# leggedrobotics/open3d_slam

Measured on AMD Instinct MI355X. Metric: icp_iterations_per_sec, higher is better.
Workload: dtype f32 points, f64 accumulate; 1 GPU; configs[1]: point-to-plane ICP, 65536-pt VLP-16 scan vs a 1,000,000-pt submap, max_corr 1.0 m, 10 fixed iterations/step (+1 evaluation pass), index prebuilt; n_src=65536, n_map_per_gpu=1000000, parallelism=1 GPU

## Files before the change

open3d_slam_amd/csrc/backend.hip:

```cpp
#include <hip/hip_runtime.h>
#include <sched.h>

#include <algorithm>
#include <atomic>
#include <chrono>
#include <cmath>
#include <cstdio>
#include <cstdlib>
#include <climits>
#include <cstring>
#include <initializer_list>
#include <map>

#include <rocprim/device/device_radix_sort.hpp>
#include <mutex>
#include <string>
#include <type_traits>
#include <unordered_map>
#include <vector>

#include "cloud_kernels.hpp"
#include "common.hpp"
#include "feature_kernels.hpp"
#include "icp_kernels.hpp"
// ... 10 lines not shown
#ifdef O3DS_AB_SWITCHES
inline const char* ab_getenv(const char* name) { return getenv(name); }
#else
inline const char* ab_getenv(const char*) { return nullptr; }
#endif

struct CloudRec {
  size_t n = 0;
  int precision = 0;
  void* pts = nullptr;
  void* nrm = nullptr;
  void* col = nullptr;
  size_t cap = 0;
  bool has_index = false;
  bool index_byproduct = false;
  GridDev grid{};
  int* cell_start = nullptr;
  void* spts = nullptr;
  void* snrm = nullptr;
  void* rpts = nullptr;
  int* rstart = nullptr;
  int* rpos = nullptr;
  int index_regs = 0;
  long long vox_first = -1;
  size_t vox_count = 0;
  struct PMapRec* pm = nullptr;
  size_t index_positions = 0;
  int lazy_slot = -1;
  int lazy_seq = 0;
  size_t n_lower = 0;
  hipEvent_t ingest_ev = nullptr;
  int ingest_buf = -1;
  int pre_slot = -1;
  int pre_seq = 0;
  CropDev pre_crop{};
  bool has_box = false;
  bool box_padded = false;
  double bmn[3] = {0, 0, 0}, bmx[3] = {0, 0, 0};
  double* fpfh = nullptr;
  bool has_fpfh = false;
  size_t fpfh_n = 0;
};

void box_inflate(CloudRec& c) {
  if (c.box_padded) return;
  c.box_padded = true;
// ... 31 lines not shown
  }
  for (int a = 0; a < 3; ++a)
    if (!std::isfinite(to.bmn[a]) || !std::isfinite(to.bmx[a])) to.has_box = false;
  if (to.has_box) box_inflate(to);
}

struct PMapRec {
  PmDev dev{};
  CropDev* d_hist = nullptr;
  int t = 0;
  size_t n_upper = 0;
  size_t live_lower = 0;
  double clamped = 0;
  double multi_total = 0;
  double pool_top = 0;
  int rec_slot = -1, rec_seq = 0;
  size_t rows = 0;
  std::vector<void*> blocks;
};

constexpr int kMaxPassBlocks = 4096;
constexpr size_t kMaxCells = (size_t)1 << 27;
constexpr size_t kReplicaMaxBytes = (size_t)256 << 20;
static_assert(kReplicaMaxBytes <= kScanMaxBytes, "scan_strided addresses a searched array by 32-bit byte offsets");

}

struct DenseRec {
  double voxel = 0.0;
  size_t cap = 0;
  o3ds::DenseDev dev{};
  bool has_normals = false;
  bool has_colors = false;
  size_t used_upper = 0;
};

struct o3ds_context {
  int device = 0;
  hipStream_t stream = nullptr;
  int precision = O3DS_PRECISION_F32;
  std::string err, deferred_err;
  std::unordered_map<uint64_t, CloudRec> clouds;
  std::unordered_map<uint64_t, DenseRec> dense_maps;
  uint64_t next_id = 1;
  double* d_partials = nullptr;
  IcpStateDev* d_state = nullptr;
// ... 355 lines not shown
}
CloudRec* find_cloud(o3ds_handle h, o3ds_cloud id) {
  auto it = h->clouds.find(id);
  if (it == h->clouds.end()) return nullptr;
  cloud_ready(h, it->second);
  if (resolve_count(h, it->second, true) != O3DS_OK || (it->second.pm && pm_exit(h, it->second) != O3DS_OK)) {
    h->deferred_err = h->err;
    return nullptr;
  }
  return &it->second;
}

void free_index(o3ds_handle h, CloudRec& c) {
  if (c.cell_start) dev_free(h, c.cell_start);
  if (c.spts) dev_free(h, c.spts);
  if (c.snrm) dev_free(h, c.snrm);
  if (c.rpts) dev_free(h, c.rpts);
  if (c.rstart) dev_free(h, c.rstart);
  if (c.rpos) dev_free(h, c.rpos);
  c.cell_start = nullptr;
  c.spts = c.snrm = c.rpts = nullptr;
  c.rstart = c.rpos = nullptr;
  c.index_regs = 0;
  c.has_index = false;
  c.index_byproduct = false;
}
constexpr int kPinRecs = 64;
inline int* cnt_word(o3ds_handle h, int slot) { return h->d_cnt + 16 * slot; }
int resolve_count(o3ds_handle h, CloudRec& c, bool block);

constexpr uint64_t kRecOwnerMap = ~0ull - 1;
int take_rec(o3ds_handle h) {
  for (int tries = 0; tries < kPinRecs; ++tries) {
    const int slot = h->rec_next;
    h->rec_next = (h->rec_next + 1) % kPinRecs;
    if (h->rec_owner[slot] == 0) {
      h->rec_owner[slot] = ~0ull;
      return slot;
    }
  }
  for (int tries = 0; tries < kPinRecs; ++tries) {
    const int slot = h->rec_next;
    h->rec_next = (h->rec_next + 1) % kPinRecs;
    auto it = h->clouds.find(h->rec_owner[slot]);
    if (it == h->clouds.end()) continue;
    if (it->second.lazy_slot == slot && resolve_count(h, it->second, true) != O3DS_OK) continue;
// ... 299 lines not shown
template <typename P4>
int bbox_of(o3ds_handle h, const P4* pts, size_t n, double mn[3], double mx[3], const CropDev* crop = nullptr) {
  const int g = grid_for(n, 1024);
  static_assert(1024 * 6 * sizeof(double) <= kPinBytes - 256, "bbox partials fit the pinned block");
  CropDev all{};
  bbox_kernel<P4><<<g, kBlock, 0, h->stream>>>(pts, n, crop ? *crop : all, (double*)h->h_pin_dev);
  HIP_TRY(hipGetLastError());
  HIP_TRY(hipStreamSynchronize(h->stream));
  const double* hb = (const double*)h->h_pin;
  for (int a = 0; a < 3; ++a) {
    mn[a] = 1e300;
    mx[a] = -1e300;
  }
  for (int b = 0; b < g; ++b)
    for (int a = 0; a < 3; ++a) {
      mn[a] = std::min(mn[a], hb[(size_t)b * 6 + a]);
      mx[a] = std::max(mx[a], hb[(size_t)b * 6 + 3 + a]);
    }
  return O3DS_OK;
}

template <typename P4>
int build_grid_t(o3ds_handle h, const P4* pts, const P4* nrm, size_t n, double cell, GridDev* out_grid, int** out_cell_start, void** out_spts,
                 void** out_snrm, CloudRec* box ,
                 const int* n_dev = nullptr ) {
  if (n == 0) return fail(h, O3DS_ERR_EMPTY, "build_index: empty cloud");
  if (n > kScanMaxBytes / sizeof(P4))
    return fail(h, O3DS_ERR_CAPACITY, "build_index: the cell-sorted points exceed 2^32 bytes (2^28 points in f32 storage, 2^27 in f64): the search addresses them by 32-bit byte offsets");
  double mn[3], mx[3];
  int rc = O3DS_OK;
  static const bool no_box_cache = ab_getenv("O3DS_NO_BOX_CACHE") != nullptr;
  if (box && box->has_box && !no_box_cache) {
    for (int a = 0; a < 3; ++a) mn[a] = box->bmn[a], mx[a] = box->bmx[a];
  } else {
    if (n_dev) return fail(h, O3DS_ERR_INVALID_ARG, "build_index: a cloud whose size is still in flight must bring its box");
    rc = bbox_of<P4>(h, pts, n, mn, mx);
    if (rc) return rc;
    if (box) {
      box->has_box = true;
      box->box_padded = false;
      for (int a = 0; a < 3; ++a) box->bmn[a] = mn[a], box->bmx[a] = mx[a];
    }
  }
  for (int a = 0; a < 3; ++a)
    if (!std::isfinite(mn[a]) || !std::isfinite(mx[a])) return fail(h, O3DS_ERR_INVALID_ARG, "build_index: non-finite coordinates");
  size_t nx, ny, nz;
  for (;;) {
    nx = (size_t)std::floor((mx[0] - mn[0]) / cell) + 1;
    ny = (size_t)std::floor((mx[1] - mn[1]) / cell) + 1;
    nz = (size_t)std::floor((mx[2] - mn[2]) / cell) + 1;
    if (nx * ny * nz <= kMaxCells) break;
    cell *= 1.26;
  }
  const size_t ncell = nx * ny * nz;
  GridDev g{};
  g.ox = mn[0];
  g.oy = mn[1];
  g.oz = mn[2];
  g.cell = cell;
  g.inv_cell = 1.0 / cell;
  g.nx = (int)nx;
  g.sx = (int)nx;
  g.ny = (int)ny;
  g.nz = (int)nz;
  int *counts = nullptr, *cell_id = nullptr, *cell_start = nullptr;
  void *spts = nullptr, *snrm = nullptr;
  rc = cell_counters(h, ncell);
  if (rc) return rc;
  if (!h->d_cells) return fail(h, O3DS_ERR_OOM, "build_index: cell counters allocation failed");
  counts = h->d_cells;
  TMP_ALLOC(cell_id, sizeof(int) * n);
  HIP_TRY(dev_alloc(h, (void**)&cell_start, sizeof(int) * (ncell + 1 + 4)));
  HIP_TRY(dev_alloc(h, (void**)&spts, sizeof(P4) * n));
  if (nrm) HIP_TRY(dev_alloc(h, (void**)&snrm, sizeof(P4) * n));
  span_mark(h, kSpanIndexBuild);
  cell_count_kernel<P4><<<grid_for(n), kBlock, 0, h->stream>>>(pts, n, g, counts, cell_id, n_dev);
  rc = exclusive_scan_int(h, counts, cell_start, ncell + 1);
  if (rc) return rc;
  scatter_kernel<P4><<<grid_for(n), kBlock, 0, h->stream>>>(pts, nrm, n, cell_id, cell_start, counts, (P4*)spts, (P4*)snrm, n_dev);
  span_mark(h, kSpanIndexBuild);
  HIP_TRY(hipGetLastError());
  h->cells_clean = true;
  dbg_sync(h, 2);
  g.cell_start = cell_start;
  *out_grid = g;
  *out_cell_start = cell_start;
  *out_spts = spts;
  if (out_snrm) *out_snrm = snrm;
  return O3DS_OK;
}

template <typename P4>
int build_index_t(o3ds_handle h, CloudRec& c, double cell) {
  free_index(h, c);
  if (c.lazy_slot >= 0 && !c.has_box) {
    const int rr = resolve_count(h, c, true);
    if (rr) return rr;
  }
  int rc = build_grid_t<P4>(h, (const P4*)c.pts, (const P4*)c.nrm, c.n, cell, &c.grid, &c.cell_start, &c.spts, &c.snrm, &c,
                            c.lazy_slot >= 0 ? cnt_word(h, c.lazy_slot) : nullptr);
  if (rc) return rc;
  c.has_index = true;
  return O3DS_OK;
}

double index_cell_div() {
  static const double d = ab_getenv("O3DS_INDEX_CELL_DIV") ? std::max(1.0, atof(ab_getenv("O3DS_INDEX_CELL_DIV"))) : 4.0;
  return d;
}

int build_index(o3ds_handle h, CloudRec& c, double cell) { return DISPATCH(c.precision, build_index_t, h, c, cell); }

template <typename P4>
int build_replica_t(o3ds_handle h, CloudRec& c) {
  GridDev g = c.grid;
  const size_t n = c.n, rcell = (size_t)g.nx * (size_t)(g.ny + 2) * (size_t)(g.nz + 2);
  if (rcell > kMaxCells || 9 * n > (size_t)INT_MAX || 9 * n * (sizeof(P4) + sizeof(int)) + sizeof(int) * (rcell + 1) > kReplicaMaxBytes) return O3DS_OK;
  void* rpts = nullptr;
  int *rstart = nullptr, *rpos = nullptr;
  if (dev_alloc(h, (void**)&rstart, sizeof(int) * (rcell + 1)) != hipSuccess || dev_alloc(h, &rpts, sizeof(P4) * 9 * n) != hipSuccess ||
      dev_alloc(h, (void**)&rpos, sizeof(int) * 9 * n) != hipSuccess) {
    (void)hipGetLastError();
    if (rstart) dev_free(h, rstart);
    if (rpts) dev_free(h, rpts);
    return O3DS_OK;
  }
  const int rs = cell_counters(h, rcell);
  if (rs || !h->d_cells) {
    (void)hipGetLastError();
    dev_free(h, rstart), dev_free(h, rpts), dev_free(h, rpos);
    return rs;
  }
  int* rcounts = h->d_cells;
  const int* n_dev = c.lazy_slot >= 0 ? cnt_word(h, c.lazy_slot) : nullptr;
  replica_count_kernel<P4><<<grid_for(n), kBlock, 0, h->stream>>>((const P4*)c.spts, n, g, rcounts, n_dev);
  const int rc = exclusive_scan_int(h, rcounts, rstart, rcell + 1);
  if (rc) {
    dev_free(h, rstart), dev_free(h, rpts), dev_free(h, rpos);
    return rc;
  }
  replica_scatter_kernel<P4><<<grid_for(n), kBlock, 0, h->stream>>>((const P4*)c.spts, n, g, rstart, rcounts, (P4*)rpts, rpos, n_dev);
  HIP_TRY(hipGetLastError());
  h->cells_clean = true;
  c.rpts = rpts;
  c.rstart = rstart;
  c.rpos = rpos;
  c.grid.rpts = rpts;
  c.grid.rstart = rstart;
  c.grid.rpos = rpos;
  return O3DS_OK;
}

constexpr int kReplicaAfterRegs = 4;
int maybe_build_replica(o3ds_handle h, CloudRec& c) {
  if (!c.has_index || c.rpts || c.pm || c.index_positions) return O3DS_OK;
  const char* e = ab_getenv("O3DS_NN_REPLICA_AFTER");
  const int after = e ? std::max(1, atoi(e)) : kReplicaAfterRegs;
  if (++c.index_regs < after) return O3DS_OK;
  return DISPATCH(c.precision, build_replica_t, h, c);
}

int h2d_copy_narrow(o3ds_handle h, float* d_dst, const double* h_src, size_t count) {
  int rc = stage_init(h);
  if (rc) return rc;
  const size_t per = kStageBytes / sizeof(float);
  int k = 0;
  for (size_t off = 0; off < count; off += per, k ^= 1) {
// ... 373 lines not shown
    int e = 0;
    (void)std::frexp(nn * bound[k], &e);
    q_hi[k] = no_split ? 0.0 : std::ldexp(1.0, e + 3 - 53);
  }
}

int begin_session(o3ds_handle h, o3ds_cloud source, o3ds_cloud target, const o3ds_crop* crop, const double init[16],
                  const o3ds_icp_params* params, bool upload_state = true) {
  CloudRec* src = find_cloud_lazy(h, source);
  CloudRec* tgt = find_cloud_lazy(h, target);
  if (src && src->pm) {
    const int re = pm_exit(h, *src);
    if (re) return re;
    tgt = find_cloud_lazy(h, target);
  }
  int rc = validate_icp(h, src, tgt, params);
  if (rc) return rc;
  const double r_hint = params->max_correspondence_distance;
  static const double reuse_max = ab_getenv("O3DS_INDEX_REUSE_MAX") ? atof(ab_getenv("O3DS_INDEX_REUSE_MAX")) : 0.75;
  if (!tgt->has_index || (tgt->nrm && !tgt->snrm) || (tgt->index_byproduct && (tgt->grid.cell < r_hint / 8.0 || tgt->grid.cell > r_hint * reuse_max))) {
    rc = build_index(h, *tgt, params->max_correspondence_distance / index_cell_div());
    if (rc) return rc;
  }
  const size_t cap = (std::max<size_t>(src->n + src->n / 4, 1 << 16) + 7) & ~(size_t)7;
  bool fresh_cache = false;
  rc = handle_scratch(h, &h->d_nn_cache, &h->nn_cache_cap, src->n, cap, cap * sizeof(int), &fresh_cache);
  if (rc) return rc;
  if (!h->d_nn_cache) return fail(h, O3DS_ERR_OOM, "icp: match cache allocation failed");
  if (fresh_cache) {
    if (h->d_set_pos) (void)hipFree(h->d_set_pos);
    h->d_set_pos = nullptr;
    h->d_set_ref = nullptr;
    if (hipMalloc((void**)&h->d_set_pos, cap * (kSetCap * sizeof(int) + 4 * sizeof(double))) != hipSuccess) {
      (void)hipFree(h->d_nn_cache);
      h->d_nn_cache = nullptr;
      h->nn_cache_cap = 0;
      return fail(h, O3DS_ERR_OOM, "icp: candidate-set allocation failed");
    }
    h->d_set_ref = (char*)h->d_set_pos + cap * kSetCap * sizeof(int);
  }
  IcpStateDev st{};
  memcpy(st.T, init, sizeof(double) * 16);
  *h->h_state = st;
  if (upload_state) HIP_TRY(hipMemcpyAsync(h->d_state, h->h_state, sizeof(IcpStateDev), hipMemcpyHostToDevice, h->stream));
  IcpPassArgs a{};
  a.src = src->pts;
  a.first = 0;
  a.count = src->n;
  a.tpts = tgt->spts;
  a.tnrm = tgt->snrm;
  rc = maybe_build_replica(h, *tgt);
  if (rc) return rc;
  a.grid = tgt->grid;
  {
    const char* e = ab_getenv("O3DS_NN_REPLICA");
    if (e && atoi(e) == 0) a.grid.rpts = nullptr, a.grid.rstart = a.grid.rpos = nullptr;
  }
  a.crop = to_dev(crop);
  const double r = params->max_correspondence_distance;
  a.r2max = r * r;
  a.method = params->method;
  record_quanta(tgt->grid, r, params->method, h->gicp_epsilon, src->n, a.q_hi);
  a.kmax = std::max(1, (int)std::ceil(r / tgt->grid.cell));
  a.nn_cache = h->d_nn_cache;
  a.set_pos = h->fused && h->sets ? h->d_set_pos : nullptr;
  a.set_ref = h->d_set_ref;
  a.set_gain = h->set_gain;
  a.set_min = h->set_min;
  a.set_cap = h->set_cap;
  a.n_tgt = (int)(tgt->index_positions ? tgt->index_positions : tgt->n);
  a.snrm = src->nrm;
  a.count_dev = src->lazy_slot >= 0 ? cnt_word(h, src->lazy_slot) : nullptr;
  a.gicp_k = 1.0 - h->gicp_epsilon;
  a.state = h->d_state;
  a.partials = h->d_partials;
// ... 1420 lines not shown
    std::vector<unsigned long long> ws((size_t)o3ds::kNrmStatWords * ((size_t)o3ds::kNrmWaves * gsz));
    HIP_TRY(hipMemcpy(ws.data(), d_ws, sizeof(unsigned long long) * ws.size(), hipMemcpyDeviceToHost));
    (void)hipFree(d_ws);
    if (FILE* f = fopen(sf, "wb")) {
      fwrite(ws.data(), sizeof(unsigned long long), ws.size(), f);
      fclose(f);
    }
  }
#endif
  if (nrm_debug) {
    fprintf(stderr, "[normals] kernel done: %s\n", hipGetErrorString(hipStreamSynchronize(h->stream)));
#ifdef O3DS_NRM_CHECK
    unsigned int dbg[8] = {0};
    (void)hipMemcpyFromSymbol(dbg, HIP_SYMBOL(o3ds::g_nrm_dbg), sizeof(dbg));
    fprintf(stderr, "[normals] violations: unsorted %u, bad p %u, bad oi %u\n", dbg[0], dbg[1], dbg[2]);
    const unsigned int zero[8] = {0};
    (void)hipMemcpyToSymbol(HIP_SYMBOL(o3ds::g_nrm_dbg), zero, sizeof(zero));
#endif
  }
  tmp.pts = nullptr;
  box_copy(c, tmp);
  free_index(h, c);
  c.grid = tmp.grid, c.cell_start = tmp.cell_start, c.spts = tmp.spts, c.snrm = tmp.snrm;
  c.has_index = true;
  c.index_byproduct = true;
  return O3DS_OK;
}

int gicp_knn_normals(o3ds_handle h, CloudRec& c) {
  return DISPATCH(c.precision, normals_t, h, c, 0.0, 20, true);
}

template <typename P4>
int transform_t(o3ds_handle h, const CloudRec& in, const double T[16], CloudRec& out) {
  out.precision = in.precision;
  out.n = in.n;
  box_transform(out, in, T);
  if (in.n == 0) return O3DS_OK;
  HIP_TRY(dev_alloc(h, (void**)&out.pts, sizeof(P4) * in.n));
  if (in.nrm) HIP_TRY(dev_alloc(h, (void**)&out.nrm, sizeof(P4) * in.n));
  transform_kernel<P4><<<grid_for(in.n), kBlock, 0, h->stream>>>((const P4*)in.pts, (const P4*)in.nrm, in.n, mat34(T), T[3], T[7], T[11], T[15],
                                                               (P4*)out.pts, (P4*)out.nrm, 0);
  if (in.col) {
    HIP_TRY(dev_alloc(h, (void**)&out.col, sizeof(P4) * in.n));
    HIP_TRY(hipMemcpyAsync(out.col, in.col, sizeof(P4) * in.n, hipMemcpyDeviceToDevice, h->stream));
  }
// ... 666 lines not shown
    if ((double)gn[0] * (double)gn[1] * (double)gn[2] <= (double)kMaxCells / 2 && gn[0] < 5000) break;
    d.kc *= 2;
    cell = d.kc * voxel;
  }
  for (int a = 0; a < 3; ++a)
    if (std::llabs(g0[a]) + gn[a] * d.kc >= (1ll << 20)) return fail(h, O3DS_ERR_INVALID_ARG, "persistent map: voxel coordinates beyond 2^20");
  d.gx0 = g0[0], d.gy0 = g0[1], d.gz0 = g0[2];
  GridDev g{};
  g.ox = (double)g0[0] * voxel;
  g.oy = (double)g0[1] * voxel;
  g.oz = (double)g0[2] * voxel;
  g.cell = cell;
  g.inv_cell = 1.0 / cell;
  g.nx = (int)gn[0], g.ny = (int)gn[1], g.nz = (int)gn[2];
  g.sx = g.nx + 1;
  pm->rows = (size_t)g.ny * g.nz;
  const size_t table = pm->rows * (size_t)g.sx;
  free_index(h, c);
  int* cs = nullptr;
  HIP_TRY(dev_alloc(h, (void**)&cs, sizeof(int) * (table + 1 + 4)));
  c.cell_start = cs;
  const size_t pool = 6 * n + 16 * scan_upper + ((size_t)1 << 22);
  if (pool >= ((size_t)1 << 31)) return fail(h, O3DS_ERR_OOM, "persistent map: index pool beyond 2^31 positions");
  if (pool > kScanMaxBytes / sizeof(P4)) return fail(h, O3DS_ERR_CAPACITY, "persistent map: index pool beyond 2^32 bytes (the search addresses it by 32-bit byte offsets)");
  HIP_TRY(dev_alloc(h, &c.spts, sizeof(P4) * pool));
  if (c.nrm) HIP_TRY(dev_alloc(h, &c.snrm, sizeof(P4) * pool));
  PM_ALLOC(d.row_cap, sizeof(int) * pm->rows);
  PM_ALLOC(d.row_flag, sizeof(int) * pm->rows);
  PM_ALLOC(d.cell_add, sizeof(int) * (table + 1));
  HIP_TRY(hipMemsetAsync(d.cell_add, 0, sizeof(int) * (table + 1), h->stream));
  g.cell_start = cs;
  d.grid = g;
  d.cs = cs;
  d.spts = c.spts;
  d.snrm = c.snrm;
  d.pool_cap = (int)pool;
  int rc = cell_counters(h, table);
  if (rc) return rc;
  if (!h->d_cells) return fail(h, O3DS_ERR_OOM, "persistent map: cell counters allocation failed");
  HIP_TRY(hipMemsetAsync(d.counters, 0, sizeof(int) * kPmCounters, h->stream));
  HIP_TRY(hipMemsetD32Async((hipDeviceptr_t)(d.counters + kPmN), (int)n, 1, h->stream));
  int* cell_id = nullptr;
  TMP_ALLOC(cell_id, sizeof(int) * n);
  const int ni = (int)n;
  span_mark(h, kSpanIndexBuild);
  pm_enter_kernel<P4><<<grid_for(n), kBlock, 0, h->stream>>>(d, ni);
  pm_cell_count_kernel<P4><<<grid_for(n), kBlock, 0, h->stream>>>(d, ni, h->d_cells, cell_id);
  pm_row_slack_kernel<<<grid_for(pm->rows * 64), kBlock, 0, h->stream>>>(h->d_cells, (int)pm->rows, g.nx, d.row_cap, d.row_flag);
// ... 1208 lines not shown
```

open3d_slam_amd/csrc/icp_kernels.hpp:

```cpp
#pragma once
#include "common.hpp"

#pragma clang fp contract(off)

namespace o3ds {

constexpr int kBlock = 256;

__device__ __forceinline__ double wave_sum(double v) {
#pragma unroll
  for (int m = 32; m >= 1; m >>= 1) v += __shfl_xor(v, m, 64);
  return v;
}
__device__ __forceinline__ float wave_min(float v) {
#pragma unroll
  for (int m = 32; m >= 1; m >>= 1) v = fminf(v, __shfl_xor(v, m, 64));
  return v;
}
__device__ __forceinline__ float wave_max(float v) {
#pragma unroll
  for (int m = 32; m >= 1; m >>= 1) v = fmaxf(v, __shfl_xor(v, m, 64));
  return v;
}

// ... 234 lines not shown
  typename Scalar<P4>::type d2;
  int pos;
  typename Scalar<P4>::index idx;
  static constexpr typename Scalar<P4>::index kNoIdx = sizeof(typename Scalar<P4>::type) == 8 ? -1 : 0;
};

template <typename R, typename I>
__device__ __forceinline__ bool nn_before(R d2, I idx, R bd2, I bidx) {
  return (d2 < bd2) | ((d2 == bd2) & (idx < bidx));
}
__device__ __forceinline__ unsigned long long nn_key(float d2, int32_t idx) {
  return ((unsigned long long)__float_as_uint(d2) << 32) | (unsigned int)idx;
}
__device__ __forceinline__ bool nn_before(float d2, int32_t idx, float bd2, int32_t bidx) { return nn_key(d2, idx) < nn_key(bd2, bidx); }

__device__ __forceinline__ float dist2(float dx, float dy, float dz) { return fmaf(dz, dz, fmaf(dy, dy, dx * dx)); }
__device__ __forceinline__ double dist2(double dx, double dy, double dz) { return dx * dx + dy * dy + dz * dz; }

template <typename P4, bool kCrop>
__device__ __forceinline__ typename Scalar<P4>::type consider(const P4& t, int p, bool valid, typename Scalar<P4>::type qx,
                                                              typename Scalar<P4>::type qy, typename Scalar<P4>::type qz,
                                                              const CropDev& crop, NNBest<P4>& best) {
  using R = typename Scalar<P4>::type;
  const R dx = t.x - qx, dy = t.y - qy, dz = t.z - qz;
  const R d2 = dist2(dx, dy, dz);
  bool better = valid & nn_before(d2, t.i, best.d2, best.idx);
  if (kCrop) {
    if (better) better = crop_contains(crop, (double)t.x, (double)t.y, (double)t.z);
  }
  best.d2 = better ? d2 : best.d2;
  best.pos = better ? p : best.pos;
  best.idx = better ? t.i : best.idx;
  return d2;
}

constexpr size_t kScanMaxBytes = (size_t)1 << 32;
constexpr int kSetCap = 4;
template <typename R>
struct Collect {
  R tau2;
  int* cnt;
  int* list;
};
template <typename R>
__device__ __forceinline__ void collect_push(const Collect<R>& c, int p) {
  const int k = atomicAdd(c.cnt, 1);
  if (k < kSetCap) c.list[k] = p;
}

template <typename P4, bool kCrop, bool kCollect, bool kRep = false>
__device__ __forceinline__ void scan_strided(const P4* __restrict__ tp, int s, int e, int lane, int stride, typename Scalar<P4>::type qx,
                                             typename Scalar<P4>::type qy, typename Scalar<P4>::type qz, const CropDev& crop,
                                             NNBest<P4>& best, const Collect<typename Scalar<P4>::type>& col) {
  using R = typename Scalar<P4>::type;
  constexpr int kInFlight = sizeof(R) == 8 ? 2 : 4;
  const char* __restrict__ tb = (const char*)tp;
  for (int p = s + lane; p < e; p += kInFlight * stride) {
    int pk[kInFlight];
    bool vk[kInFlight];
    P4 tk[kInFlight];
    R dk[kInFlight];
#pragma unroll
    for (int k = 0; k < kInFlight; ++k) {
      pk[k] = p + k * stride;
      vk[k] = pk[k] < e;
      tk[k] = *(const P4*)(tb + (unsigned)(vk[k] ? pk[k] : p) * (unsigned)sizeof(P4));
    }
    if (sizeof(R) == 8) __builtin_amdgcn_sched_barrier(0);
#pragma unroll
    for (int k = 0; k < kInFlight; ++k) dk[k] = consider<P4, kCrop>(tk[k], pk[k], vk[k], qx, qy, qz, crop, best);
    if (kCollect) {
      R dmin = dk[0];
#pragma unroll
      for (int k = 1; k < kInFlight; ++k) dmin = min(dmin, dk[k]);
      if (dmin < col.tau2) {
#pragma unroll
        for (int k = 0; k < kInFlight; ++k)
          if (vk[k] & (dk[k] < col.tau2)) collect_push(col, kRep ? -2 - pk[k] : pk[k]);
      }
    }
  }
}

template <typename P4, int W>
__device__ __forceinline__ void lanes_min(NNBest<P4>& b) {
#pragma unroll
  for (int m = 1; m < W; m <<= 1) {
    const auto od2 = __shfl_xor(b.d2, m, W);
    const int opos = __shfl_xor(b.pos, m, W);
    const auto oidx = __shfl_xor(b.idx, m, W);
    const bool take = (opos != -1) & nn_before(od2, oidx, b.d2, b.idx);
    b.d2 = take ? od2 : b.d2;
    b.pos = take ? opos : b.pos;
    b.idx = take ? oidx : b.idx;
  }
}

constexpr int kFarList = 256;
constexpr int kSegMax = 32;

__device__ __forceinline__ void lds_barrier() { asm volatile("s_waitcnt lgkmcnt(0)\n\ts_barrier" ::: "memory"); }

__device__ __forceinline__ void lds_wave_sync() {
  __builtin_amdgcn_fence(__ATOMIC_RELEASE, "wavefront");
  __builtin_amdgcn_wave_barrier();
  __builtin_amdgcn_fence(__ATOMIC_ACQUIRE, "wavefront");
}

template <int G>
__device__ __forceinline__ int group_exclusive_sum(int c, int gl, int* total) {
  int incl = c;
#pragma unroll
  for (int d = 1; d < G; d <<= 1) {
    const int o = __shfl_up(incl, d, G);
    if (gl >= d) incl += o;
  }
  *total = __shfl(incl, G - 1, G);
  return incl - c;
}

struct QueryCell {
  float ux, uy, uz;
  float mf;
  int ix, iy, iz;
};

__device__ __forceinline__ QueryCell locate(const GridDev& g, double qx, double qy, double qz) {
  QueryCell c;
  const double fx = (qx - g.ox) * g.inv_cell, fy = (qy - g.oy) * g.inv_cell, fz = (qz - g.oz) * g.inv_cell;
  const double flx = floor(fx), fly = floor(fy), flz = floor(fz);
  const double lim = 1.0e9;
  c.ix = (int)fmin(fmax(flx, -lim), lim);
  c.iy = (int)fmin(fmax(fly, -lim), lim);
  c.iz = (int)fmin(fmax(flz, -lim), lim);
  c.ux = (float)(fx - flx);
  c.uy = (float)(fy - fly);
  c.uz = (float)(fz - flz);
  c.mf = fminf(fminf(fminf(c.ux, 1.0f - c.ux), fminf(c.uy, 1.0f - c.uy)), fminf(c.uz, 1.0f - c.uz));
  return c;
}
// ... 43 lines not shown
  const int* __restrict__ cs = g.cell_start;
  const int xlo = max(c.ix - 1, 0), xhi = min(c.ix + 1, g.nx - 1);
  if (g.rpts) {
    const P4* __restrict__ rp = (const P4*)g.rpts;
    const bool sv = xlo <= xhi && (unsigned)(c.iy + 1) < (unsigned)(g.ny + 2) && (unsigned)(c.iz + 1) < (unsigned)(g.nz + 2);
    const int srow = sv ? ((c.iz + 1) * (g.ny + 2) + (c.iy + 1)) * g.nx : 0;
    int v[4];
#pragma unroll
    for (int j = 0; j < 4; ++j) v[j] = sv ? g.rstart[srow + min(xlo + j, xhi + 1)] : 0;
    lanes_min<P4, G>(best);
    const int pos0 = best.pos;
    const auto idx0 = best.idx;
    const float b2 = bound_cells2(best.d2, m, g);
    int s = 0, e = 0, xa, xb;
    if (sv && row_extent(b2, 0.0f, c.ux, &xa, &xb)) {
      xa = max(c.ix + xa, xlo);
      xb = min(c.ix + xb, xhi);
      if (xa <= xb) {
        const int ja = xa - xlo, jb = xb - xlo + 1;
        s = ja == 0 ? v[0] : (ja == 1 ? v[1] : v[2]);
        e = jb == 1 ? v[1] : (jb == 2 ? v[2] : v[3]);
      }
    }
    scan_strided<P4, kCrop, kCollect, true>(rp, s, e, gl, G, qx, qy, qz, crop, best, col);
    lanes_min<P4, G>(best);
    if (best.pos != -1 && !(pos0 != -1 && best.idx == idx0)) best.pos = g.rpos[best.pos];
  } else {
    constexpr int kOwn = (9 + G - 1) / G;
    int v[kOwn][4];
    bool rv[kOwn];
#pragma unroll
    for (int k = 0; k < kOwn; ++k) {
      const int r = gl + k * G, rz = div3_row(r);
      const int y = c.iy + (r - 3 * rz) - 1, z = c.iz + rz - 1;
      rv[k] = r < 9 && xlo <= xhi && (unsigned)y < (unsigned)g.ny && (unsigned)z < (unsigned)g.nz;
      const int* __restrict__ rowp = cs + (rv[k] ? (z * g.ny + y) * g.sx : 0);
#pragma unroll
      for (int j = 0; j < 4; ++j) v[k][j] = rv[k] ? row_entry(rowp, min(xlo + j, xhi + 1)) : 0;
    }
    {
      const float b2 = bound_cells2(best.d2, m, g);
      int ss[kOwn], ee[kOwn];
      int cnt = 0;
#pragma unroll
      for (int k = 0; k < kOwn; ++k) {
        const int r = gl + k * G, rz = div3_row(r);
        const float ddy = slab_dist((r - 3 * rz) - 1, c.uy), ddz = slab_dist(rz - 1, c.uz);
        int xa, xb;
        ss[k] = ee[k] = 0;
        if (rv[k] && row_extent(b2, ddy * ddy + ddz * ddz, c.ux, &xa, &xb)) {
          xa = max(c.ix + xa, xlo);
          xb = min(c.ix + xb, xhi);
          if (xa <= xb) {
            const int ja = xa - xlo, jb = xb - xlo + 1;
            ss[k] = ja == 0 ? v[k][0] : (ja == 1 ? v[k][1] : v[k][2]);
            ee[k] = jb == 1 ? v[k][1] : (jb == 2 ? v[k][2] : v[k][3]);
          }
        }
        cnt += ee[k] > ss[k] ? 1 : 0;
      }
      int total;
      int off = group_exclusive_sum<G>(cnt, gl, &total);
#pragma unroll
      for (int k = 0; k < kOwn; ++k)
        if (ee[k] > ss[k]) seg[off++] = make_int2(ss[k], ee[k]);
      lds_wave_sync();
      for (int t = 0; t < total; ++t) {
        const int2 se = seg[t];
        scan_strided<P4, kCrop, kCollect>(tp, se.x, se.y, gl, G, qx, qy, qz, crop, best, col);
      }
      lds_wave_sync();
      lanes_min<P4, G>(best);
    }
  }
  const float ic2 = (float)(g.inv_cell * g.inv_cell) * (1.0f + 1e-4f);
  bool proven = kmax <= 1 || widen2(best.d2, m) * ic2 <= (1.0f + c.mf) * (1.0f + c.mf);
  *kdone = 1;
  if (!proven) {
    constexpr int kHalf = 13, kOwn2 = (kHalf + G - 1) / G;
#pragma unroll 1
    for (int r0 = 0; r0 < 25; r0 += kHalf) {
      const float b2 = bound_cells2(best.d2, m, g);
      const int own = min(kHalf, 25 - r0);
      int s2[2 * kOwn2], e2[2 * kOwn2];
#pragma unroll
      for (int k = 0; k < kOwn2; ++k) {
        const int rl = gl + k * G, r = r0 + rl, rz = div5_row(r);
        const int dy = (r - 5 * rz) - 2, dz = rz - 2;
        const int y = c.iy + dy, z = c.iz + dz;
        const float ddy = slab_dist(dy, c.uy), ddz = slab_dist(dz, c.uz);
        int xa, xb;
        const bool reach = row_extent(b2, ddy * ddy + ddz * ddz, c.ux, &xa, &xb) && rl < own && (unsigned)y < (unsigned)g.ny &&
                           (unsigned)z < (unsigned)g.nz;
        xa = max(c.ix + max(xa, -2), 0);
        xb = min(c.ix + min(xb, 2), g.nx - 1);
        const bool inner = abs(dy) <= 1 && abs(dz) <= 1;
        const int* __restrict__ rowp = cs + (reach ? (z * g.ny + y) * g.sx : 0);
        const int xb1 = inner ? min(xb, c.ix - 2) : xb, xa2 = max(xa, c.ix + 2);
        const bool h0 = reach && xa <= xb1, h1 = reach && inner && xa2 <= xb;
        s2[2 * k] = row_entry(rowp, h0 ? xa : 0);
        e2[2 * k] = row_entry(rowp, h0 ? xb1 + 1 : 0);
        s2[2 * k + 1] = row_entry(rowp, h1 ? xa2 : 0);
        e2[2 * k + 1] = row_entry(rowp, h1 ? xb + 1 : 0);
      }
      int cnt = 0;
#pragma unroll
      for (int k = 0; k < 2 * kOwn2; ++k) cnt += e2[k] > s2[k] ? 1 : 0;
      int total;
      int off = group_exclusive_sum<G>(cnt, gl, &total);
#pragma unroll
      for (int k = 0; k < 2 * kOwn2; ++k)
        if (e2[k] > s2[k]) seg[off++] = make_int2(s2[k], e2[k]);
      lds_wave_sync();
      for (int t = 0; t < total; ++t) {
        const int2 se = seg[t];
        scan_strided<P4, kCrop, kCollect>(tp, se.x, se.y, gl, G, qx, qy, qz, crop, best, col);
      }
      lds_wave_sync();
      lanes_min<P4, G>(best);
    }
    proven = kmax <= 2 || widen2(best.d2, m) * ic2 <= (2.0f + c.mf) * (2.0f + c.mf);
    *kdone = 2;
  }
  *resolved = proven;
  return best;
}

__device__ __forceinline__ int far_side_recip(int K) { return (65536 + 2 * K) / (2 * K + 1); }

template <typename P4, bool kCrop, bool kCollect>
__device__ __forceinline__ void nn_search_wave_far(const GridDev& g, const P4* __restrict__ tp, typename Scalar<P4>::type qx,
                                                   typename Scalar<P4>::type qy, typename Scalar<P4>::type qz, int K,
                                                   const CropDev& crop, NNBest<P4>& best, int lane, int side_recip ,
                                                   int2* s_list , typename Scalar<P4>::type m,
                                                   const Collect<typename Scalar<P4>::type>& col) {
  constexpr int kdone = 2;
  constexpr int kPer = 4;
  const QueryCell c = locate(g, (double)qx, (double)qy, (double)qz);
  const float b2 = bound_cells2(best.d2, m, g);
// ... 158 lines not shown
  const int qw = ql % kQPW;
  if (order == 2) {
    const size_t n_run = (count + kQPW - 1) / kQPW;
    const size_t run = n_run % kMul ? (size_t)(((unsigned long long)off * kMul) % n_run) : off;
    const size_t i = run * kQPW + (size_t)qw;
    return off < n_run && i < count ? i : count;
  }
  constexpr int kRun = 1, kRuns = kQPW / kRun;
  static_assert(kQPW % kRun == 0, "runs tile a wavefront");
  const size_t n_run = (count + kRun - 1) / kRun;
  const size_t n_off = (n_run + kRuns - 1) / kRuns;
  const size_t offs = n_off % kMul ? (size_t)(((unsigned long long)off * kMul) % n_off) : off;
  const size_t run = (size_t)(qw / kRun) * n_off + offs;
  const size_t i = run * kRun + (size_t)(qw % kRun);
  return off < n_off && run < n_run && i < count ? i : count;
}

__host__ __device__ __forceinline__ int pass_order(int pass) { return pass == 0 ? 1 : (pass == 1 ? 2 : 0); }

template <typename P4>
struct QueryPrefetch {
  P4 s, tprev;
  int prev;
  P4 nprev;
  typename Scalar<P4>::type rx, ry, rz, rL;
};

template <typename P4>
struct alignas(4 * sizeof(typename Scalar<P4>::type)) SetRef {
  typename Scalar<P4>::type x, y, z, L;
};

__device__ __forceinline__ size_t deal_count(const IcpPassArgs& a) { return a.count_dev ? min((size_t)*a.count_dev, a.count) : a.count; }

template <typename P4, int kPassBlock, int kGroup>
__device__ __forceinline__ QueryPrefetch<P4> prefetch_query(const IcpPassArgs& a, size_t batch, bool use_cache, bool use_sets, int order, size_t n_deal) {
  constexpr int kQPB = kPassBlock / kGroup;
  using R = typename Scalar<P4>::type;
  QueryPrefetch<P4> q;
  q.prev = -1;
  q.s = P4{};
  q.nprev = P4{};
  q.tprev = P4{};
  q.rx = q.ry = q.rz = q.rL = (R)0;
  const bool sets = use_cache && use_sets && a.set_pos != nullptr;
  const size_t i = query_index<kQPB, 64 / kGroup>(n_deal, batch, threadIdx.x / kGroup, order);
  if (a.count == 0) return q;
  static_assert(sizeof(SetRef<P4>) == sizeof(P4), "a source point stands in for the reference a mode without sets does not read");
  static_assert(kGroup == kSetCap, "one listed point per lane of the group");
  const bool live = i < a.count;
  const size_t ic = a.first + (live ? i : a.count - 1);
  const P4* __restrict__ src = (const P4*)a.src;
  const int* pprev = sets ? a.set_pos + ic * kSetCap + (threadIdx.x & (kGroup - 1)) : a.nn_cache + ic;
  const SetRef<P4>* pref = sets ? (const SetRef<P4>*)a.set_ref + ic : (const SetRef<P4>*)(src + ic);
  const P4 s = src[ic];
  int prev = *pprev;
  const SetRef<P4> r = *pref;
  if (prev >= a.n_tgt || !live || !use_cache) prev = -1;
  const int pc = max(prev, 0);
  const P4 t = ((const P4*)a.tpts)[pc];
  const P4 nrm = ((const P4*)(sets && a.tnrm ? a.tnrm : a.tpts))[pc];
  q.s = s;
  q.prev = prev;
  q.tprev = t;
  q.nprev = nrm;
  q.rx = r.x, q.ry = r.y, q.rz = r.z, q.rL = sets && live ? r.L : (R)0;
  return q;
}

// ... 75 lines not shown
  const P4* __restrict__ tn = (const P4*)a.tnrm;
  const double t00 = to_sgpr(Tm[0]), t10 = to_sgpr(Tm[1]), t20 = to_sgpr(Tm[2]), t01 = to_sgpr(Tm[4]), t11 = to_sgpr(Tm[5]),
               t21 = to_sgpr(Tm[6]), t02 = to_sgpr(Tm[8]), t12 = to_sgpr(Tm[9]), t22 = to_sgpr(Tm[10]), t03 = to_sgpr(Tm[12]),
               t13 = to_sgpr(Tm[13]), t23 = to_sgpr(Tm[14]);
  const int gl = threadIdx.x & (kGroup - 1), ql = threadIdx.x / kGroup;
  const int term = threadIdx.x & 31, qs = threadIdx.x >> 5;
  const bool inf = a.method == kMethodInformation;
  const bool p2p = a.method == O3DS_ICP_POINT_TO_POINT || inf;
  const int ta = term_slot(inf ? kPackA_inf.lo : (p2p ? kPackA_p2p.lo : kPackA.lo), inf ? kPackA_inf.hi : (p2p ? kPackA_p2p.hi : kPackA.hi), term);
  const int tb = term_slot(inf ? kPackB_inf.lo : (p2p ? kPackB_p2p.lo : kPackB.lo), inf ? kPackB_inf.hi : (p2p ? kPackB_p2p.hi : kPackB.hi), term);
  const bool sets = !kKeys && a.set_pos != nullptr && s_set != nullptr;
  const bool sets_in = sets && use_cache;
  const bool sets_out = kCollect && sets;
  const R rmax = (R)sqrt(a.r2max);
  int* my_set = sets ? s_set + ql * (1 + kSetCap) : nullptr;
  double acc = 0.0;
  const size_t n_batches = (n_live + kQPB - 1) / kQPB;
  static_assert(sizeof(FarItem<P4>) <= kStride * sizeof(double), "a parked far query fits its record slot");
  static_assert((2 + kQPB) * sizeof(int) <= (kPassBlock / 32) * kRec * sizeof(double), "the far list fits s_red");
  int* s_far = (int*)&s_red[0][0];
  if (threadIdx.x == 0) s_far[0] = s_far[1] = 0;
  lds_barrier();
  for (size_t b = (size_t)wg; b < n_batches; b += kSingle ? n_batches : (size_t)nwg) {
    const size_t i = query_index<kQPB, 64 / kGroup>(n_live, b, ql, order);
    double px = 0, py = 0, pz = 0;
    NNBest<P4> nn;
    nn.pos = -1;
    nn.idx = -1;
    nn.d2 = (R)0;
    bool unresolved = false;
    bool verified = false;
    int kdone = 0;
    R m = (R)0;
    const QueryPrefetch<P4> qp = (kSingle || b == (size_t)wg) ? first_batch : prefetch_query<P4, kPassBlock, kGroup>(a, b, use_cache, sets, order, n_live);
    if (sets && gl == 0) my_set[0] = 0;
    if (i < n_live) {
      const P4 s = qp.s;
      px = t00 * (double)s.x + t01 * (double)s.y + t02 * (double)s.z + t03;
      py = t10 * (double)s.x + t11 * (double)s.y + t12 * (double)s.z + t13;
      pz = t20 * (double)s.x + t21 * (double)s.y + t22 * (double)s.z + t23;
      const R qx = (R)px, qy = (R)py, qz = (R)pz;
      bool resolved = true;
      if (a.debug == 2) {
        nn.pos = (int)(i % 1000);
        nn.idx = nn.pos;
      } else if (kKeys && a.keys_mode == 2) {
        const unsigned long long key = a.keys[a.first + i];
// ... 900 lines not shown
```

open3d_slam_amd/csrc/map_kernels.hpp:

```cpp
#pragma once
#include "cloud_kernels.hpp"
#include "common.hpp"

namespace o3ds {

#pragma clang fp contract(off)

constexpr int kPmHistory = 256;
constexpr unsigned long long kPmRaw = 1ull << 63;
constexpr unsigned int kPmDead = 1, kPmUnsettled = 2, kPmFresh = 4, kPmCarved = 8;
constexpr int kPmMaxOld = 8;

struct alignas(32) PmSlot {
  unsigned long long okey;
  int stamp;
  int pos;
  int hnext;
  unsigned int flags;
  int out_tau;
  int out_checked;
};
struct alignas(16) PmHash {
  unsigned long long key;
  int head;
// ... 249 lines not shown
        l = t == 0 ? (unsigned long long)s : (st == t ? ok : kp);
      } else if ((ok & kPmRaw) && st > 0) {
        h = ((unsigned long long)st << 1) | 1ull;
        l = ok & ~kPmRaw;
      } else {
        h = 0;
        l = (unsigned long long)s;
      }
    }
    if (lane == leader) *hi = h, *lo = l;
  }
}

__global__ __launch_bounds__(kBlock) void pm_hash_init_kernel(PmHash* __restrict__ hh, size_t n) {
  for (size_t i = (size_t)blockIdx.x * kBlock + threadIdx.x; i < n; i += (size_t)gridDim.x * kBlock) {
    PmHash e;
    e.key = kEmptyKey;
    e.head = -1;
    e.info = 0u;
    hh[i] = e;
  }
}
template <typename P4>
__global__ __launch_bounds__(kBlock) void pm_enter_kernel(PmDev m, int n) {
  int* err = m.counters + kPmError;
  for (int s = blockIdx.x * kBlock + threadIdx.x; s < n; s += gridDim.x * kBlock) {
    const P4 p = ((const P4*)m.pts)[s];
    const unsigned long long k = pm_key(p, m.inv_voxel);
    m.slot[s].stamp = 0;
    m.slot[s].okey = k;
    m.slot[s].out_checked = -1;
    m.slot[s].out_tau = 0;
    unsigned int fl = 0;
    if (m.nrm) {
      const P4 nv = ((const P4*)m.nrm)[s];
      if (!pm_same_bits(pm_renormalized(nv), nv)) {
        fl |= kPmUnsettled;
        pm_push(m.unsettled[0], m.counters + kPmUnsettledIn, m.list_cap, s, err);
      }
    }
    m.slot[s].flags = fl;
    const unsigned int e = pm_entry(m, k);
    const int old = atomicExch(&m.h[e].head, s);
    m.slot[s].hnext = old;
    if (old != -1 && !(atomicOr(&m.h[e].info, 1u) & 1u)) pm_push64(m.multi[0], m.counters + kPmMultiOut, m.list_cap, k, err);
  }
// ... 1050 lines not shown
```

Before: 58800 icp_iterations/s.

## Pad scan arrays with slack, use constant-stride loads and DPP/permlane lane reductions

Adds a 4 KiB slack tail to the cell-sorted and replica point arrays so the strided scan loop can issue unconditional loads at compile-time stride offsets instead of clamping each address. The nearest-neighbour lane reduction and the group prefix sum now use DPP and permlane swaps in place of generic shuffles. Several smaller pieces ride along: the single-batch path reuses the prefetched query index, the f32 distance uses a paired float subtraction, and the persistent-map pool is cleared to far sentinels. The cost is extra memory, a check that ICP targets carry the slack, a replica build moved earlier, and reliance on gfx950-specific permlane builtins.

```diff
diff --git a/open3d_slam_amd/csrc/backend.hip b/open3d_slam_amd/csrc/backend.hip
--- a/open3d_slam_amd/csrc/backend.hip
+++ b/open3d_slam_amd/csrc/backend.hip
@@ -56,6 +56,8 @@
   int* rstart = nullptr;
   int* rpos = nullptr;
   int index_regs = 0;
+  size_t spts_slack = 0;
+  size_t rpts_slack = 0;
   long long vox_first = -1;
   size_t vox_count = 0;
   struct PMapRec* pm = nullptr;
@@ -133,6 +135,14 @@
 constexpr int kMaxPassBlocks = 4096;
 constexpr size_t kMaxCells = (size_t)1 << 27;
 constexpr size_t kReplicaMaxBytes = (size_t)256 << 20;
+template <typename P4>
+size_t scan_capacity() {
+  static_assert(kScanMaxBytes + kScanSlackBytes == (size_t)1 << 32, "capacity and slack share the 32-bit offset space");
+  const char* e = ab_getenv("O3DS_SCAN_SPACE_BYTES");
+  const size_t space = e ? (size_t)strtoull(e, nullptr, 10) : kScanMaxBytes + kScanSlackBytes;
+  return space > kScanSlackBytes ? (std::min(space, kScanMaxBytes + kScanSlackBytes) - kScanSlackBytes) / sizeof(P4) : 0;
+}
+inline size_t scan_slack_alloc() { return ab_getenv("O3DS_NO_SCAN_SLACK") ? 0 : kScanSlackBytes; }
 static_assert(kReplicaMaxBytes <= kScanMaxBytes, "scan_strided addresses a searched array by 32-bit byte offsets");
 
 }
@@ -534,6 +544,7 @@
   c.spts = c.snrm = c.rpts = nullptr;
   c.rstart = c.rpos = nullptr;
   c.index_regs = 0;
+  c.spts_slack = c.rpts_slack = 0;
   c.has_index = false;
   c.index_byproduct = false;
 }
@@ -879,11 +890,12 @@
 
 template <typename P4>
 int build_grid_t(o3ds_handle h, const P4* pts, const P4* nrm, size_t n, double cell, GridDev* out_grid, int** out_cell_start, void** out_spts,
-                 void** out_snrm, CloudRec* box ,
+                 void** out_snrm, size_t* out_slack ,
+                 CloudRec* box ,
                  const int* n_dev = nullptr ) {
   if (n == 0) return fail(h, O3DS_ERR_EMPTY, "build_index: empty cloud");
-  if (n > kScanMaxBytes / sizeof(P4))
-    return fail(h, O3DS_ERR_CAPACITY, "build_index: the cell-sorted points exceed 2^32 bytes (2^28 points in f32 storage, 2^27 in f64): the search addresses them by 32-bit byte offsets");
+  if (n > scan_capacity<P4>())
+    return fail(h, O3DS_ERR_CAPACITY, "build_index: the cell-sorted points exceed 2^32 bytes less the scan loop's slack (the search addresses them by 32-bit byte offsets)");
   double mn[3], mx[3];
   int rc = O3DS_OK;
   static const bool no_box_cache = ab_getenv("O3DS_NO_BOX_CACHE") != nullptr;
@@ -928,7 +940,8 @@
   counts = h->d_cells;
   TMP_ALLOC(cell_id, sizeof(int) * n);
   HIP_TRY(dev_alloc(h, (void**)&cell_start, sizeof(int) * (ncell + 1 + 4)));
-  HIP_TRY(dev_alloc(h, (void**)&spts, sizeof(P4) * n));
+  const size_t slack = scan_slack_alloc();
+  HIP_TRY(dev_alloc(h, (void**)&spts, sizeof(P4) * n + slack));
   if (nrm) HIP_TRY(dev_alloc(h, (void**)&snrm, sizeof(P4) * n));
   span_mark(h, kSpanIndexBuild);
   cell_count_kernel<P4><<<grid_for(n), kBlock, 0, h->stream>>>(pts, n, g, counts, cell_id, n_dev);
@@ -943,6 +956,7 @@
   *out_grid = g;
   *out_cell_start = cell_start;
   *out_spts = spts;
+  *out_slack = slack;
   if (out_snrm) *out_snrm = snrm;
   return O3DS_OK;
 }
@@ -954,7 +968,7 @@
     const int rr = resolve_count(h, c, true);
     if (rr) return rr;
   }
-  int rc = build_grid_t<P4>(h, (const P4*)c.pts, (const P4*)c.nrm, c.n, cell, &c.grid, &c.cell_start, &c.spts, &c.snrm, &c,
+  int rc = build_grid_t<P4>(h, (const P4*)c.pts, (const P4*)c.nrm, c.n, cell, &c.grid, &c.cell_start, &c.spts, &c.snrm, &c.spts_slack, &c,
                             c.lazy_slot >= 0 ? cnt_word(h, c.lazy_slot) : nullptr);
   if (rc) return rc;
   c.has_index = true;
@@ -975,7 +989,7 @@
   if (rcell > kMaxCells || 9 * n > (size_t)INT_MAX || 9 * n * (sizeof(P4) + sizeof(int)) + sizeof(int) * (rcell + 1) > kReplicaMaxBytes) return O3DS_OK;
   void* rpts = nullptr;
   int *rstart = nullptr, *rpos = nullptr;
-  if (dev_alloc(h, (void**)&rstart, sizeof(int) * (rcell + 1)) != hipSuccess || dev_alloc(h, &rpts, sizeof(P4) * 9 * n) != hipSuccess ||
+  if (dev_alloc(h, (void**)&rstart, sizeof(int) * (rcell + 1)) != hipSuccess || dev_alloc(h, &rpts, sizeof(P4) * 9 * n + scan_slack_alloc()) != hipSuccess ||
       dev_alloc(h, (void**)&rpos, sizeof(int) * 9 * n) != hipSuccess) {
     (void)hipGetLastError();
     if (rstart) dev_free(h, rstart);
@@ -1000,6 +1014,7 @@
   HIP_TRY(hipGetLastError());
   h->cells_clean = true;
   c.rpts = rpts;
+  c.rpts_slack = scan_slack_alloc();
   c.rstart = rstart;
   c.rpos = rpos;
   c.grid.rpts = rpts;
@@ -1419,6 +1434,10 @@
     rc = build_index(h, *tgt, params->max_correspondence_distance / index_cell_div());
     if (rc) return rc;
   }
+  rc = maybe_build_replica(h, *tgt);
+  if (rc) return rc;
+  if (tgt->spts_slack < kScanSlackBytes || (tgt->rpts && tgt->rpts_slack < kScanSlackBytes))
+    return fail(h, O3DS_ERR_INVALID_ARG, "icp: the target's index arrays end without the kScanSlackBytes the search's scan loop may load beyond a range");
   const size_t cap = (std::max<size_t>(src->n + src->n / 4, 1 << 16) + 7) & ~(size_t)7;
   bool fresh_cache = false;
   rc = handle_scratch(h, &h->d_nn_cache, &h->nn_cache_cap, src->n, cap, cap * sizeof(int), &fresh_cache);
@@ -1446,8 +1465,6 @@
   a.count = src->n;
   a.tpts = tgt->spts;
   a.tnrm = tgt->snrm;
-  rc = maybe_build_replica(h, *tgt);
-  if (rc) return rc;
   a.grid = tgt->grid;
   {
     const char* e = ab_getenv("O3DS_NN_REPLICA");
@@ -2914,6 +2931,7 @@
   box_copy(c, tmp);
   free_index(h, c);
   c.grid = tmp.grid, c.cell_start = tmp.cell_start, c.spts = tmp.spts, c.snrm = tmp.snrm;
+  c.spts_slack = tmp.spts_slack;
   c.has_index = true;
   c.index_byproduct = true;
   return O3DS_OK;
@@ -3626,8 +3644,13 @@
   c.cell_start = cs;
   const size_t pool = 6 * n + 16 * scan_upper + ((size_t)1 << 22);
   if (pool >= ((size_t)1 << 31)) return fail(h, O3DS_ERR_OOM, "persistent map: index pool beyond 2^31 positions");
-  if (pool > kScanMaxBytes / sizeof(P4)) return fail(h, O3DS_ERR_CAPACITY, "persistent map: index pool beyond 2^32 bytes (the search addresses it by 32-bit byte offsets)");
-  HIP_TRY(dev_alloc(h, &c.spts, sizeof(P4) * pool));
+  if (pool > scan_capacity<P4>()) return fail(h, O3DS_ERR_CAPACITY, "persistent map: index pool beyond 2^32 bytes less the scan loop's slack (the search addresses it by 32-bit byte offsets)");
+  HIP_TRY(dev_alloc(h, &c.spts, sizeof(P4) * pool + scan_slack_alloc()));
+  c.spts_slack = scan_slack_alloc();
+  {
+    const size_t n_clear = pool + c.spts_slack / sizeof(P4);
+    pm_pool_clear_kernel<P4><<<(unsigned)std::min<size_t>((n_clear + kBlock - 1) / kBlock, 8192), kBlock, 0, h->stream>>>((P4*)c.spts, n_clear);
+  }
   if (c.nrm) HIP_TRY(dev_alloc(h, &c.snrm, sizeof(P4) * pool));
   PM_ALLOC(d.row_cap, sizeof(int) * pm->rows);
   PM_ALLOC(d.row_flag, sizeof(int) * pm->rows);
diff --git a/open3d_slam_amd/csrc/icp_kernels.hpp b/open3d_slam_amd/csrc/icp_kernels.hpp
--- a/open3d_slam_amd/csrc/icp_kernels.hpp
+++ b/open3d_slam_amd/csrc/icp_kernels.hpp
@@ -280,7 +280,15 @@
                                                               typename Scalar<P4>::type qy, typename Scalar<P4>::type qz,
                                                               const CropDev& crop, NNBest<P4>& best) {
   using R = typename Scalar<P4>::type;
-  const R dx = t.x - qx, dy = t.y - qy, dz = t.z - qz;
+  R dx, dy;
+  if constexpr (sizeof(R) == 4) {
+    typedef float f32x2 __attribute__((ext_vector_type(2)));
+    const f32x2 d = f32x2{t.x, t.y} - f32x2{qx, qy};
+    dx = d.x, dy = d.y;
+  } else {
+    dx = t.x - qx, dy = t.y - qy;
+  }
+  const R dz = t.z - qz;
   const R d2 = dist2(dx, dy, dz);
   bool better = valid & nn_before(d2, t.i, best.d2, best.idx);
   if (kCrop) {
@@ -292,7 +300,6 @@
   return d2;
 }
 
-constexpr size_t kScanMaxBytes = (size_t)1 << 32;
 constexpr int kSetCap = 4;
 template <typename R>
 struct Collect {
@@ -306,23 +313,31 @@
   if (k < kSetCap) c.list[k] = p;
 }
 
-template <typename P4, bool kCrop, bool kCollect, bool kRep = false>
+constexpr size_t kScanSlackBytes = 4096;
+constexpr size_t kScanMaxBytes = ((size_t)1 << 32) - kScanSlackBytes;
+
+template <typename P4, bool kCrop, bool kCollect, bool kRep = false, int kStride = 0>
 __device__ __forceinline__ void scan_strided(const P4* __restrict__ tp, int s, int e, int lane, int stride, typename Scalar<P4>::type qx,
                                              typename Scalar<P4>::type qy, typename Scalar<P4>::type qz, const CropDev& crop,
                                              NNBest<P4>& best, const Collect<typename Scalar<P4>::type>& col) {
   using R = typename Scalar<P4>::type;
   constexpr int kInFlight = sizeof(R) == 8 ? 2 : 4;
+  static_assert((kInFlight - 1) * 64 * sizeof(P4) <= kScanSlackBytes && kStride <= 64, "what a batch loads beyond the end of a range lies in the slack");
+  const int st = kStride ? kStride : stride;
   const char* __restrict__ tb = (const char*)tp;
-  for (int p = s + lane; p < e; p += kInFlight * stride) {
+  for (int p = s + lane; p < e; p += kInFlight * st) {
     int pk[kInFlight];
     bool vk[kInFlight];
     P4 tk[kInFlight];
     R dk[kInFlight];
 #pragma unroll
     for (int k = 0; k < kInFlight; ++k) {
-      pk[k] = p + k * stride;
+      pk[k] = p + k * st;
       vk[k] = pk[k] < e;
-      tk[k] = *(const P4*)(tb + (unsigned)(vk[k] ? pk[k] : p) * (unsigned)sizeof(P4));
+      if (kStride)
+        tk[k] = *(const P4*)(tb + (size_t)((unsigned)p * (unsigned)sizeof(P4)) + (size_t)k * kStride * sizeof(P4));
+      else
+        tk[k] = *(const P4*)(tb + (unsigned)pk[k] * (unsigned)sizeof(P4));
     }
     if (sizeof(R) == 8) __builtin_amdgcn_sched_barrier(0);
 #pragma unroll
@@ -340,17 +355,92 @@
   }
 }
 
+constexpr int kDppQuadXor1 = 0xB1;
+constexpr int kDppQuadXor2 = 0x4E;
+constexpr int kDppQuadShr1 = 0x90;
+constexpr int kDppQuadShr2 = 0x40;
+constexpr int kDppQuadLane3 = 0xFF;
+constexpr int kDppRowHalfMirror = 0x141;
+constexpr int kDppRowMirror = 0x140;
+template <int kCtrl>
+__device__ __forceinline__ int dpp_move(int v) {
+  return __builtin_amdgcn_update_dpp(0, v, kCtrl, 0xF, 0xF, true);
+}
+template <int kCtrl>
+__device__ __forceinline__ float dpp_move(float v) {
+  return __int_as_float(dpp_move<kCtrl>(__float_as_int(v)));
+}
+template <int kCtrl>
+__device__ __forceinline__ double dpp_move(double v) {
+  return __hiloint2double(dpp_move<kCtrl>(__double2hiint(v)), dpp_move<kCtrl>(__double2loint(v)));
+}
+template <int kCtrl>
+__device__ __forceinline__ int64_t dpp_move(int64_t v) {
+  const unsigned lo = (unsigned)dpp_move<kCtrl>((int)(unsigned)v), hi = (unsigned)dpp_move<kCtrl>((int)(unsigned)((uint64_t)v >> 32));
+  return (int64_t)(((uint64_t)hi << 32) | lo);
+}
+
+template <typename P4>
+__device__ __forceinline__ void nn_take(NNBest<P4>& b, typename Scalar<P4>::type od2, int opos, typename Scalar<P4>::index oidx) {
+  const bool take = (opos != -1) & nn_before(od2, oidx, b.d2, b.idx);
+  b.d2 = take ? od2 : b.d2;
+  b.pos = take ? opos : b.pos;
+  b.idx = take ? oidx : b.idx;
+}
+template <typename P4, int kCtrl>
+__device__ __forceinline__ void nn_take_dpp(NNBest<P4>& b) {
+  nn_take<P4>(b, dpp_move<kCtrl>(b.d2), dpp_move<kCtrl>(b.pos), dpp_move<kCtrl>(b.idx));
+}
+template <bool k32>
+__device__ __forceinline__ void lane_swap(int v, int* a, int* b) {
+  const auto r = k32 ? __builtin_amdgcn_permlane32_swap((unsigned)v, (unsigned)v, false, false)
+                     : __builtin_amdgcn_permlane16_swap((unsigned)v, (unsigned)v, false, false);
+  *a = (int)r[0], *b = (int)r[1];
+}
+template <bool k32>
+__device__ __forceinline__ void lane_swap(float v, float* a, float* b) {
+  int ia, ib;
+  lane_swap<k32>(__float_as_int(v), &ia, &ib);
+  *a = __int_as_float(ia), *b = __int_as_float(ib);
+}
+template <bool k32>
+__device__ __forceinline__ void lane_swap(double v, double* a, double* b) {
+  int la, lb, ha, hb;
+  lane_swap<k32>(__double2loint(v), &la, &lb);
+  lane_swap<k32>(__double2hiint(v), &ha, &hb);
+  *a = __hiloint2double(ha, la), *b = __hiloint2double(hb, lb);
+}
+template <bool k32>
+__device__ __forceinline__ void lane_swap(int64_t v, int64_t* a, int64_t* b) {
+  int la, lb, ha, hb;
+  lane_swap<k32>((int)(unsigned)v, &la, &lb);
+  lane_swap<k32>((int)(unsigned)((uint64_t)v >> 32), &ha, &hb);
+  *a = (int64_t)(((uint64_t)(unsigned)ha << 32) | (unsigned)la), *b = (int64_t)(((uint64_t)(unsigned)hb << 32) | (unsigned)lb);
+}
+template <typename P4, bool k32>
+__device__ __forceinline__ void nn_take_swap(NNBest<P4>& b) {
+  NNBest<P4> lo, hi;
+  lane_swap<k32>(b.d2, &lo.d2, &hi.d2);
+  lane_swap<k32>(b.pos, &lo.pos, &hi.pos);
+  lane_swap<k32>(b.idx, &lo.idx, &hi.idx);
+  nn_take<P4>(lo, hi.d2, hi.pos, hi.idx);
+  b = lo;
+}
+
 template <typename P4, int W>
 __device__ __forceinline__ void lanes_min(NNBest<P4>& b) {
-#pragma unroll
-  for (int m = 1; m < W; m <<= 1) {
-    const auto od2 = __shfl_xor(b.d2, m, W);
-    const int opos = __shfl_xor(b.pos, m, W);
-    const auto oidx = __shfl_xor(b.idx, m, W);
-    const bool take = (opos != -1) & nn_before(od2, oidx, b.d2, b.idx);
-    b.d2 = take ? od2 : b.d2;
-    b.pos = take ? opos : b.pos;
-    b.idx = take ? oidx : b.idx;
+  if constexpr (W == 4 || W == 64) {
+    nn_take_dpp<P4, kDppQuadXor1>(b);
+    nn_take_dpp<P4, kDppQuadXor2>(b);
+    if constexpr (W == 64) {
+      nn_take_dpp<P4, kDppRowHalfMirror>(b);
+      nn_take_dpp<P4, kDppRowMirror>(b);
+      nn_take_swap<P4, false>(b);
+      nn_take_swap<P4, true>(b);
+    }
+  } else {
+#pragma unroll
+    for (int m = 1; m < W; m <<= 1) nn_take<P4>(b, __shfl_xor(b.d2, m, W), __shfl_xor(b.pos, m, W), __shfl_xor(b.idx, m, W));
   }
 }
 
@@ -368,12 +458,20 @@
 template <int G>
 __device__ __forceinline__ int group_exclusive_sum(int c, int gl, int* total) {
   int incl = c;
-#pragma unroll
-  for (int d = 1; d < G; d <<= 1) {
-    const int o = __shfl_up(incl, d, G);
-    if (gl >= d) incl += o;
-  }
-  *total = __shfl(incl, G - 1, G);
+  if constexpr (G == 4) {
+    const int o1 = dpp_move<kDppQuadShr1>(incl);
+    if (gl >= 1) incl += o1;
+    const int o2 = dpp_move<kDppQuadShr2>(incl);
+    if (gl >= 2) incl += o2;
+    *total = dpp_move<kDppQuadLane3>(incl);
+  } else {
+#pragma unroll
+    for (int d = 1; d < G; d <<= 1) {
+      const int o = __shfl_up(incl, d, G);
+      if (gl >= d) incl += o;
+    }
+    *total = __shfl(incl, G - 1, G);
+  }
   return incl - c;
 }
 
@@ -463,7 +561,7 @@
         e = jb == 1 ? v[1] : (jb == 2 ? v[2] : v[3]);
       }
     }
-    scan_strided<P4, kCrop, kCollect, true>(rp, s, e, gl, G, qx, qy, qz, crop, best, col);
+    scan_strided<P4, kCrop, kCollect, true, G>(rp, s, e, gl, G, qx, qy, qz, crop, best, col);
     lanes_min<P4, G>(best);
     if (best.pos != -1 && !(pos0 != -1 && best.idx == idx0)) best.pos = g.rpos[best.pos];
   } else {
@@ -508,7 +606,7 @@
       lds_wave_sync();
       for (int t = 0; t < total; ++t) {
         const int2 se = seg[t];
-        scan_strided<P4, kCrop, kCollect>(tp, se.x, se.y, gl, G, qx, qy, qz, crop, best, col);
+        scan_strided<P4, kCrop, kCollect, false, G>(tp, se.x, se.y, gl, G, qx, qy, qz, crop, best, col);
       }
       lds_wave_sync();
       lanes_min<P4, G>(best);
@@ -555,7 +653,7 @@
       lds_wave_sync();
       for (int t = 0; t < total; ++t) {
         const int2 se = seg[t];
-        scan_strided<P4, kCrop, kCollect>(tp, se.x, se.y, gl, G, qx, qy, qz, crop, best, col);
+        scan_strided<P4, kCrop, kCollect, false, G>(tp, se.x, se.y, gl, G, qx, qy, qz, crop, best, col);
       }
       lds_wave_sync();
       lanes_min<P4, G>(best);
@@ -760,6 +858,7 @@
 struct QueryPrefetch {
   P4 s, tprev;
   int prev;
+  unsigned qi;
   P4 nprev;
   typename Scalar<P4>::type rx, ry, rz, rL;
 };
@@ -783,6 +882,7 @@
   q.rx = q.ry = q.rz = q.rL = (R)0;
   const bool sets = use_cache && use_sets && a.set_pos != nullptr;
   const size_t i = query_index<kQPB, 64 / kGroup>(n_deal, batch, threadIdx.x / kGroup, order);
+  q.qi = (unsigned)i;
   if (a.count == 0) return q;
   static_assert(sizeof(SetRef<P4>) == sizeof(P4), "a source point stands in for the reference a mode without sets does not read");
   static_assert(kGroup == kSetCap, "one listed point per lane of the group");
@@ -904,7 +1004,7 @@
   if (threadIdx.x == 0) s_far[0] = s_far[1] = 0;
   lds_barrier();
   for (size_t b = (size_t)wg; b < n_batches; b += kSingle ? n_batches : (size_t)nwg) {
-    const size_t i = query_index<kQPB, 64 / kGroup>(n_live, b, ql, order);
+    const size_t i = kSingle ? (size_t)first_batch.qi : query_index<kQPB, 64 / kGroup>(n_live, b, ql, order);
     double px = 0, py = 0, pz = 0;
     NNBest<P4> nn;
     nn.pos = -1;
diff --git a/open3d_slam_amd/csrc/map_kernels.hpp b/open3d_slam_amd/csrc/map_kernels.hpp
--- a/open3d_slam_amd/csrc/map_kernels.hpp
+++ b/open3d_slam_amd/csrc/map_kernels.hpp
@@ -295,6 +295,15 @@
   }
 }
 template <typename P4>
+__global__ __launch_bounds__(kBlock) void pm_pool_clear_kernel(P4* __restrict__ pool, size_t n) {
+  using R = typename Scalar<P4>::type;
+  P4 far;
+  far.x = far.y = far.z = sizeof(R) == 4 ? (R)3.0e38f : (R)1.0e300;
+  far.i = (typename Scalar<P4>::index)0x7fffffff;
+  for (size_t i = (size_t)blockIdx.x * kBlock + threadIdx.x; i < n; i += (size_t)gridDim.x * kBlock) pool[i] = far;
+}
+
+template <typename P4>
 __global__ __launch_bounds__(kBlock) void pm_enter_kernel(PmDev m, int n) {
   int* err = m.counters + kPmError;
   for (int s = blockIdx.x * kBlock + threadIdx.x; s < n; s += gridDim.x * kBlock) {
```

After: 60940 icp_iterations/s, median of 6. 1.04x the previous value.
